# kije/gpu_raytracer

Hardware: AMD Instinct MI355X
Metric: Mrays/s (higher is better)
Workload: dtype f32

## Files before the change

gpu_raytracer_amd/csrc/rt_frame.cpp:

```cpp
#include "rt_internal.h"

#ifndef RT_SINGLE_PASS_MAX_NODES
#define RT_SINGLE_PASS_MAX_NODES 64u
#endif
#ifndef RT_WF_LANES_DEFAULT
#define RT_WF_LANES_DEFAULT 2
#endif

namespace rti {
DevCamera make_camera(const rt_camera& cam, float res_x, float res_y, bool wavefront) {
    DevCamera c;
    float wf, hf;
    if (wavefront) {
        wf = res_x;
        hf = res_y;
    } else {
        auto as_u32 = [](float f) -> uint32_t { return !(f > 0.0f) ? 0u : (f >= 4294967296.0f ? 0xFFFFFFFFu : (uint32_t)f); };
        wf = (float)as_u32(res_x);
        hf = (float)as_u32(res_y);
    }
    c.width_f = wf;
    c.height_f = hf;
    c.aspect = wf / hf;
    c.fov_scale = tanf(cam.fov * 0.5f * 3.14159265358979323846f / 180.0f);
// ... 311 lines not shown
    if (two) {
        HIPCHK(ctx, hipEventRecord(d.ev_start, d.stream));
        HIPCHK(ctx, hipStreamWaitEvent(d.stream2, d.ev_start, 0));
        HIPCHK(ctx, hipMemsetAsync(d.pipe.wf2.totals, 0, rt::WF_N_TOTALS * sizeof(unsigned long long), d.stream2));
    }
    d.pipe.wf.grids = d.pipe.wf2.grids = (f.flags & RT_FLAG_NO_SHADOW_GRID) ? nullptr : d.grids.table.get();
    const char* pe = std::getenv("RT_WF_PROBE");
    d.pipe.wf.probe = d.pipe.wf2.probe = pe ? (uint32_t)std::atoi(pe) : 0u;
    d.used_two_lanes = two;
    r = WfRun{};
    r.phase = WfRun::GENERATE;
    r.pipeline = true;
    r.dev = j;
    r.f = f;
    r.dsc = scene_for(ctx, d);
    r.batch = batch;
    r.n_blocks = n_blocks;
    r.two = two;
    r.beams = beams;
    return RT_OK;
}

struct WfLane { rt::WfBuffers w; hipStream_t st; };
WfLane lane_of(const DeviceState& d, const WfRun& r) {
    const bool second = r.two && (r.j & 1u);
    WfLane l{second ? d.pipe.wf2 : d.pipe.wf, second ? d.stream2 : d.stream};
    if (!r.beams) l.w.beam_count = nullptr;
    l.w.n_blocks = r.n_blocks;
    l.w.batch = r.batch;
    return l;
}
uint32_t batch_samples(const WfRun& r) { return std::min(r.batch, r.f.spp - r.first); }

int wf_step_generate(rt_ctx* ctx, DeviceState& d, WfRun& r, const WfLane& l) {
    HIPCHK(ctx, rt::wf_generate(r.dsc, r.f, l.w, targets_for(d, r.f), r.first, batch_samples(r), l.st));
    r.it = 0;
    r.phase = WfRun::BOUNCE;
    return RT_OK;
}

int wf_step_bounce(rt_ctx* ctx, DeviceState& d, WfRun& r, const WfLane& l, bool counters, std::vector<WfRun*>& polls) {
    hipEvent_t* gev = nullptr;
    if ((r.f.flags & RT_FLAG_STAGE_TIMES) && r.dev == 0 && rt::wf_runs_shadow_grid(r.f, l.w)) {
        if (d.stage_events.size() < (size_t)d.stage_events_used + 2) {
            hipEvent_t a = nullptr, b = nullptr;
            HIPCHK(ctx, hipEventCreate(&a));
            HIPCHK(ctx, hipEventCreate(&b));
            d.stage_events.push_back(a);
            d.stage_events.push_back(b);
        }
        gev = d.stage_events.data() + d.stage_events_used;
        d.stage_events_used += 2;
    }
    HIPCHK(ctx, rt::wf_bounce(r.dsc, r.f, l.w, r.it, batch_samples(r), counters, l.st, gev));
    if (r.it >= r.f.max_bounce) r.phase = WfRun::RESOLVE;
    else if ((r.it & 7u) == 7u) {
        HIPCHK(ctx, hipMemcpyAsync(&r.alive, l.w.counters + rt::WF_EXT_COUNT, 4, hipMemcpyDeviceToHost, l.st));
        r.poll_stream = l.st;
        polls.push_back(&r);
    } else r.it++;
    return RT_OK;
}

int wf_step_resolve(rt_ctx* ctx, DeviceState& d, WfRun& r, const WfLane& l) {
    const uint32_t n = batch_samples(r);
    if (r.two && r.j > 0) HIPCHK(ctx, hipStreamWaitEvent(l.st, d.ev_res[(r.j - 1u) & 1u], 0));
    HIPCHK(ctx, rt::wf_resolve(r.f, l.w, targets_for(d, r.f), n, r.first, r.first == 0, r.first + n >= r.f.spp, l.st));
    if (r.two) HIPCHK(ctx, hipEventRecord(d.ev_res[r.j & 1u], l.st));
    r.first += r.batch;
    r.j++;
    if (r.first < r.f.spp) {
        r.phase = WfRun::GENERATE;
        return RT_OK;
    }
    if (r.two) {
        HIPCHK(ctx, hipEventRecord(d.ev_join, d.stream2));
        HIPCHK(ctx, hipStreamWaitEvent(d.stream, d.ev_join, 0));
    }
    if (r.f.adaptive) HIPCHK(ctx, rt::launch_ad_image(r.f, targets_for(d, r.f), d.stream));
    HIPCHK(ctx, hipEventRecord(d.ev1, d.stream));
    r.phase = WfRun::DONE;
    return RT_OK;
}

struct FrameTotals {
    double kernel_ms = 0.0;
    uint64_t pixels = 0;
    unsigned long long segments = 0, camera = 0, continuation = 0, shadow = 0, node_visits = 0, tri_tests = 0;
    unsigned long long diag[RT_CNT_N_DIAG] = {0};
    unsigned long long grid_answered = 0, grid_entries = 0;
};

void add_counters(FrameTotals& t, const unsigned long long (&c)[RT_CNT_SLOTS]) {
    t.segments += c[RT_CNT_SEGMENTS], t.camera += c[RT_CNT_CAMERA], t.continuation += c[RT_CNT_CONTINUATION], t.shadow += c[RT_CNT_SHADOW];
    t.node_visits += c[RT_CNT_NODE_VISITS], t.tri_tests += c[RT_CNT_TRI_TESTS];
    for (int k = 0; k < RT_CNT_N_DIAG; k++) t.diag[k] += c[RT_CNT_DIAG + k];
}

void merge_lanes(unsigned long long (&t)[rt::WF_N_TOTALS], const unsigned long long (&t2)[rt::WF_N_TOTALS]) {
    for (int k = 0; k < rt::WF_N_TOTALS; k++) t[k] = k == rt::WF_TOTAL_STACK_MAX ? std::max(t[k], t2[k]) : t[k] + t2[k];
}

int add_totals(rt_ctx* ctx, FrameTotals& t, const unsigned long long (&w)[rt::WF_N_TOTALS]) {
    t.segments += w[rt::WF_TOTAL_CAMERA] + w[rt::WF_TOTAL_CONTINUATION] + w[rt::WF_TOTAL_SHADOW];
    t.camera += w[rt::WF_TOTAL_CAMERA], t.continuation += w[rt::WF_TOTAL_CONTINUATION], t.shadow += w[rt::WF_TOTAL_SHADOW];
    t.node_visits += w[rt::WF_TOTAL_NODE_VISITS], t.tri_tests += w[rt::WF_TOTAL_TRI_TESTS];
    if (w[rt::WF_TOTAL_ERROR] != 0)
// ... 273 lines not shown
```

gpu_raytracer_amd/csrc/wavefront.h:

```cpp
#ifndef RT_WAVEFRONT_H
#define RT_WAVEFRONT_H

#include <hip/hip_runtime.h>

#include "../../include/rt_hip.h"
#include "device_layout.h"
#include "shadow_grid.h"

namespace rt {

enum WfCounter : uint32_t {
    WF_EXT_COUNT = 0,
    WF_EXT_NEXT = 1,
    WF_SHADOW2_COUNT = 2,
    WF_SHADOW_COUNT = 3,
    WF_EXT_CURSOR = 4,
    WF_SHADOW_CURSOR = 5,
    WF_EXT_WINDOW = 6,
    WF_SHADOW_WINDOW = 7,
    WF_EXT_WINDOW_NEXT = 8,
    WF_SHADOW2_CURSOR = 9,
    WF_SHADOW2_WINDOW = 10,
    WF_UNUSED_11 = 11,
    WF_FB_COUNT = 12,
// ... 24 lines not shown
struct WfBuffers {
    float4* ray_o;
    float4* ray_d;
    float4* thr;
    float4* rad;
    float4* next_o;
    float4* next_d;
    float4* next_thr;
    float4* next_rad;
    float4* vtx;
    float4* sample_rad;
    uint32_t* pxy;
    uint32_t* q_ext[2];
    uint32_t* q_shadow;
    uint32_t* q_shadow2;
    const DevShadowGrid* grids;
    uint32_t* counters;
    unsigned long long* totals;
    float4* accum;
    uint32_t q_ext_cap;
    uint32_t q_shadow_cap;
    uint32_t state_cap;
    uint32_t* stack_ovf;
    uint32_t ovf_entries;
    uint32_t n_blocks;
    uint32_t batch;
    uint32_t capacity;
    uint32_t* beam_count;
    uint32_t* beam_ref;
    float* beam_dist;
    uint32_t probe;
};

#ifndef RT_BEAM_CAP
#define RT_BEAM_CAP 128u
#endif
#define RT_BEAM_OVERFLOW 0x80000000u
#ifndef RT_WF8_LDS_STACK
#define RT_WF8_LDS_STACK 8
#endif
#define RT_WF_MAX_LIGHTS 32u
#define RT_WF_ID_MASK 0x07FFFFFFu

uint32_t wf_shading_blocks();
size_t wf_state_slots(size_t paths);
size_t wf_state_slots_for(size_t paths, size_t producing_waves);
size_t wf_queue_slots(size_t max_entries, uint32_t per_lane);
size_t wf_queue_slots_for(size_t max_entries, uint32_t per_lane, size_t producing_waves);
uint32_t wf_pick_window(uint32_t iterations, uint32_t per_lane);
uint32_t wf_persistent_waves();
hipError_t wf_beams(const DevScene& sc, const DevFrame& fr, const WfBuffers& wb, hipStream_t s);
hipError_t wf_generate(const DevScene& sc, const DevFrame& fr, const WfBuffers& wb, const DevTargets& tg, uint32_t first_sample, uint32_t n_samples, hipStream_t s);
inline bool wf_runs_shadow_grid(const DevFrame& fr, const WfBuffers& wb) { return !(fr.flags & RT_FLAG_NO_SHADOWS) && wb.grids; }
hipError_t wf_bounce(const DevScene& sc, const DevFrame& fr, const WfBuffers& wb, uint32_t iteration, uint32_t n_samples, bool counters, hipStream_t s,
                     hipEvent_t* grid_events = nullptr);
hipError_t wf_resolve(const DevFrame& fr, const WfBuffers& wb, const DevTargets& tg, uint32_t n_samples, uint32_t first_sample, bool first_batch, bool last_batch,
                      hipStream_t s);

}
#endif
```

gpu_raytracer_amd/csrc/wavefront.hip:

```cpp
#include "wavefront.h"
#include <cstdlib>

#include <algorithm>

#include "device_common.h"
#include "shadow_grid_walk.h"

using namespace rtdev;

#ifndef RT_WF_REFILL
#define RT_WF_REFILL 16
#endif
#ifndef RT_WF_CHUNK
#define RT_WF_CHUNK 256
#endif
#ifndef RT_WF_ADAPTIVE_CHUNK
#define RT_WF_ADAPTIVE_CHUNK 1
#endif
#ifndef RT_WF_WINDOW
#define RT_WF_WINDOW 512
#endif
#ifndef RT_WF_BLOCK_MAJOR
#define RT_WF_BLOCK_MAJOR 1
#endif
// ... 20 lines not shown

#ifndef RT_WF_WINDOW_MAX
#define RT_WF_WINDOW_MAX 16384u
#endif
__host__ __device__ inline uint32_t wf_min_window(uint32_t per_lane) {
    uint32_t w = RT_WF_WINDOW;
    while (w < 128u * per_lane) w <<= 1;
    return w;
}
__host__ __device__ inline uint32_t pick_window(uint32_t iters, uint32_t per_lane) {
    const uint32_t most = iters * WAVE * per_lane;
    uint32_t w = wf_min_window(per_lane);
    while (w < most / 4u && w < RT_WF_WINDOW_MAX) w <<= 1;
    return w;
}
struct OutWindow {
    uint32_t next, end;
};
#define WF_SENTINEL 0xFFFFFFFFu
__device__ __forceinline__ void window_close(uint32_t* __restrict__ queue, OutWindow& w) {
    for (uint32_t i = w.next + (threadIdx.x & 63u); i < w.end; i += WAVE) queue[i] = WF_SENTINEL;
    w.next = w.end;
}
#define WF_NO_SLOT 0xFFFFFFFFu
__device__ __forceinline__ uint32_t window_reserve(uint32_t* __restrict__ queue, uint32_t* __restrict__ counter, OutWindow& w, uint32_t window,
                                                  uint32_t mine, uint32_t incl, uint32_t total, uint32_t capacity, unsigned long long* __restrict__ error) {
    if (w.next + total > w.end) {
        window_close(queue, w);
        uint32_t base = 0;
        if ((threadIdx.x & 63u) == 0) base = atomicAdd(counter, window);
        base = __shfl(base, 0, WAVE);
        if (base > capacity || window > capacity - base) {
            if ((threadIdx.x & 63u) == 0) atomicOr(error, 1ull);
            w.next = w.end = 0u;
            return WF_NO_SLOT;
        }
        w.next = base;
        w.end = base + window;
    }
    const uint32_t at = w.next + incl - mine;
    w.next += total;
    return at;
}
__device__ __forceinline__ uint32_t wave_incl_scan(uint32_t v) {
    const uint32_t lane = threadIdx.x & 63u;
#pragma unroll
    for (int off = 1; off < WAVE; off <<= 1) {
        const uint32_t u = __shfl_up(v, off, WAVE);
        if ((int)lane >= off) v += u;
    }
    return v;
}

template <bool AD>
__global__ __launch_bounds__(256) void k_wf_generate(DevFrame fr, rt::WfBuffers wb, DevTargets tg, uint32_t first_sample, uint32_t n_slots_blocks) {
    const uint32_t lane = threadIdx.x & 63u;
    const uint32_t n_waves = gridDim.x * 4u, wave = blockIdx.x * 4u + (threadIdx.x >> 6);
    OutWindow win = {0u, 0u};
    uint32_t real = 0;
    const uint32_t window = pick_window((n_slots_blocks + n_waves - 1u) / n_waves, 1u);
    if (blockIdx.x == 0 && threadIdx.x == 0) {
        wb.counters[rt::WF_EXT_WINDOW] = window;
        if (wb.beam_count) wb.counters[rt::WF_FB_COUNT] = wb.beam_count[wb.n_blocks] * (n_slots_blocks / max(1u, wb.n_blocks)) * WAVE;
    }
    const uint32_t n_samples = n_slots_blocks / max(1u, wb.n_blocks);
    for (uint32_t sb = wave; sb < n_slots_blocks; sb += n_waves) {
#if RT_WF_BLOCK_MAJOR
        const uint32_t b = sb / n_samples, k = sb - b * n_samples;
#else
        const uint32_t k = sb / wb.n_blocks, b = sb - k * wb.n_blocks;
#endif
        PixelCoord px = block_pixel_at(fr, AD ? fr.ad_blocks[b] : b, lane);
        uint32_t base = fr.sample_base;
        if (AD) {
            px.valid = px.valid && ad_lane_active(fr, fr.ad_blocks[b], lane);
            if (px.valid) base = ad_load(fr, tg, (size_t)px.y * fr.width + px.x).n;
        }
        const uint32_t p = sb * WAVE + lane;
        if (px.valid) {
            V3 o, d;
            const SimpleRng rng = ext_sample_ray(fr.cam, fr.width, fr.frame_seed, fr.jitter, px.x, px.y, base + first_sample + k, true, o, d);
            wb.ray_o[p] = make_float4(o.x, o.y, o.z, 0.0f);
            wb.ray_d[p] = make_float4(d.x, d.y, d.z, __uint_as_float(p));
            wb.thr[p] = make_float4(1.0f, 1.0f, 1.0f, __uint_as_float(3u));
            wb.rad[p] = make_float4(0.0f, 0.0f, 0.0f, __uint_as_float(rng.seed));
            wb.pxy[p] = px.x | (px.y << 16);
        } else {
            wb.pxy[p] = 0xFFFFFFFFu;
            wb.sample_rad[p] = make_float4(0.0f, 0.0f, 0.0f, 0.0f);
        }
        const uint32_t mine = px.valid ? 1u : 0u;
        const uint32_t incl = wave_incl_scan(mine), total = __shfl(incl, WAVE - 1, WAVE);
        if (total) {
            const uint32_t at = window_reserve(wb.q_ext[0], &wb.counters[rt::WF_EXT_COUNT], win, window, mine, incl, total, wb.q_ext_cap, &wb.totals[rt::WF_TOTAL_ERROR]);
            if (mine && at != WF_NO_SLOT) wb.q_ext[0][at] = p;
            real += mine;
        }
        if (wb.beam_count) {
            const uint32_t bc = wb.beam_count[b];
            if (bc & RT_BEAM_OVERFLOW) wb.q_ext[1][((size_t)(bc & ~RT_BEAM_OVERFLOW) * n_samples + k) * WAVE + lane] = px.valid ? p : WF_SENTINEL;
        }
    }
    window_close(wb.q_ext[0], win);
    const unsigned long long r = wave_sum(real);
    if (lane == 0 && r) atomicAdd(&wb.totals[rt::WF_TOTAL_CAMERA], r);
}

#ifndef RT_WF8_LDS_STACK
#define RT_WF8_LDS_STACK 8
#endif
#ifndef RT_WF8_MIN_WAVES
#define RT_WF8_MIN_WAVES 6
#endif
#ifndef RT_WF8_LEAF_THRESHOLD
#define RT_WF8_LEAF_THRESHOLD 24
#endif
#define WF8_KIND_T 0x80000000u
#define WF8_NONE 0xFFFFFFFFu

#define WF_NO_VERTEX 0xFFFFFFFFu
#define WF_END_SKY 0u
#define WF_END_MAGENTA 1u
__device__ __forceinline__ uint32_t wf_all_lights(uint32_t n_lights) { return n_lights >= RT_WF_MAX_LIGHTS ? 0xFFFFFFFFu : (1u << n_lights) - 1u; }
__device__ __forceinline__ void wf_store_vertex(const DevScene& sc, const rt::WfBuffers& wb, uint32_t id, bool found, V3 point, V3 normal, uint32_t material_id) {
    float4* __restrict__ rec = wb.vtx + 2 * (size_t)id;
    if (found && material_id < sc.n_materials) {
        rec[0] = make_float4(point.x, point.y, point.z, __uint_as_float(material_id));
        rec[1] = make_float4(normal.x, normal.y, normal.z, __uint_as_float(wf_all_lights(sc.n_lights)));
    } else {
        rec[0] = make_float4(__uint_as_float(found ? WF_END_MAGENTA : WF_END_SKY), 0.0f, 0.0f, __uint_as_float(WF_NO_VERTEX));
    }
}

template <bool COUNT, bool ANY>
__global__ __launch_bounds__(WAVE, RT_WF8_MIN_WAVES) void k_wf_trace(DevScene sc, rt::WfBuffers wb, const uint32_t* __restrict__ queue, uint32_t count_slot,
                                                    uint32_t cursor_slot, uint32_t window_slot) {
    extern __shared__ uint32_t s_mem8[];
    if (wb.totals[rt::WF_TOTAL_ERROR] != 0ull) return;
    const uint32_t lane = threadIdx.x;
    uint2* __restrict__ stack = reinterpret_cast<uint2*>(s_mem8) + lane;
    uint8_t* __restrict__ lut = reinterpret_cast<uint8_t*>(s_mem8 + RT_WF8_LDS_STACK * 2 * WAVE);
    for (uint32_t e = lane; e < 2048u; e += WAVE) {
        const uint32_t oct = e >> 8, m = e & 255u;
        uint32_t best = 0u, best_key = 99u;
        for (uint32_t i = 0; i < 8u; i++)
            if (((m >> i) & 1u) && (i ^ oct) < best_key) best_key = i ^ oct, best = i;
        lut[e] = (uint8_t)best;
    }
    __syncthreads();
    uint2* __restrict__ ovf = reinterpret_cast<uint2*>(wb.stack_ovf) + (size_t)blockIdx.x * wb.ovf_entries * WAVE + lane;
    const uint4* __restrict__ nodes = reinterpret_cast<const uint4*>(sc.nodes);
    const uint32_t count = wb.counters[count_slot];
// ... 349 lines not shown
    for (uint32_t l0 = 0; l0 < n_leaf && !overflow; l0 += WAVE) {
        const uint32_t li = l0 + lane;
        uint32_t first = 0, count = 0;
        if (li < n_leaf) {
            first = s_leaf[li];
            count = sc.tris[first].leaf_count;
        }
        for (uint32_t k = 0; k < RT_DEV_LEAF_STRIDE; k++) {
            bool keep = false;
            float dist = 0.0f;
            if (k < count) {
                const DevTri& t = sc.tris[first + k];
                float lo[3], hi[3];
                for (int a = 0; a < 3; a++) {
                    const float va = t.v0[a], vb = t.v0[a] + t.e1[a], vc = t.v0[a] + t.e2[a];
                    lo[a] = fminf(va, fminf(vb, vc));
                    hi[a] = fmaxf(va, fmaxf(vb, vc));
                    const float pad = (fabsf(lo[a]) + fabsf(hi[a])) * 2.0e-6f + 1.0e-30f;
                    lo[a] -= pad;
                    hi[a] += pad;
                }
                keep = !RT_BEAM_TRI_CULL || !(lo[0] <= hi[0] && lo[1] <= hi[1] && lo[2] <= hi[2]) || !beam_outside(bp, lo, hi);
                dist = beam_box_distance(bp.o, lo, hi);
                if (!(dist >= 0.0f)) dist = 0.0f;
            }
            const unsigned long long mk = __ballot(keep);
            const uint32_t pos = n_tri + (uint32_t)__popcll(mk & lower);
            if (keep && pos < RT_BEAM_CAP) {
                s_ref[pos] = first + k;
                s_dist[pos] = dist;
            }
            n_tri += (uint32_t)__popcll(mk);
        }
        overflow = n_tri > RT_BEAM_CAP;
    }
    __syncthreads();
    if (overflow) {
        if (lane == 0) wb.beam_count[b] = RT_BEAM_OVERFLOW | atomicAdd(&wb.beam_count[wb.n_blocks], 1u);
        return;
    }
    for (uint32_t i = lane; i < n_tri; i += WAVE) {
        const float di = s_dist[i];
        uint32_t rank = 0;
        for (uint32_t j = 0; j < n_tri; j++) {
            const float dj = s_dist[j];
            rank += (dj < di || (dj == di && j < i)) ? 1u : 0u;
        }
        wb.beam_ref[(size_t)b * RT_BEAM_CAP + rank] = s_ref[i];
        wb.beam_dist[(size_t)b * RT_BEAM_CAP + rank] = di;
    }
    if (lane == 0) wb.beam_count[b] = n_tri;
}

template <bool COUNT>
__global__ __launch_bounds__(WAVE) void k_wf_trace_camera(DevScene sc, rt::WfBuffers wb, uint32_t n_samples) {
    extern __shared__ uint4 s_cam[];
    if (wb.totals[rt::WF_TOTAL_ERROR] != 0ull) return;
    const uint32_t lane = threadIdx.x;
    float* s_d = reinterpret_cast<float*>(s_cam + RT_BEAM_CAP * 3u);
    Counts cnt = {0u, 0u};
    const uint32_t chunks = (n_samples + RT_BEAM_SAMPLES_PER_WAVE - 1u) / RT_BEAM_SAMPLES_PER_WAVE;
    for (uint32_t item = blockIdx.x; item < wb.n_blocks * chunks; item += gridDim.x) {
        const uint32_t b = item / chunks, k_first = (item - b * chunks) * RT_BEAM_SAMPLES_PER_WAVE, k_end = min(n_samples, k_first + RT_BEAM_SAMPLES_PER_WAVE);
        const uint32_t n_list = (uint32_t)__builtin_amdgcn_readfirstlane((int)wb.beam_count[b]);
        if (n_list & RT_BEAM_OVERFLOW) continue;
        {
            __syncthreads();
            for (uint32_t i = lane; i < n_list; i += WAVE) {
                const uint32_t slot = wb.beam_ref[(size_t)b * RT_BEAM_CAP + i];
                const uint4* __restrict__ rec = reinterpret_cast<const uint4*>(sc.tris + slot);
                const uint4 q0 = rec[0], q1 = rec[1], q2 = rec[2];
                s_cam[3u * i] = q0;
                s_cam[3u * i + 1u] = q1;
                s_cam[3u * i + 2u] = make_uint4(q2.x, q2.y, q2.z, slot);
                s_d[i] = wb.beam_dist[(size_t)b * RT_BEAM_CAP + i];
            }
            __syncthreads();
        }
        for (uint32_t k = k_first; k < k_end; k++) {
            const uint32_t sb = RT_WF_BLOCK_MAJOR ? b * n_samples + k : k * wb.n_blocks + b;
            const uint32_t p = sb * WAVE + lane;
            const bool valid = wb.pxy[p] != 0xFFFFFFFFu;
            if (__ballot(valid) == 0ull) continue;
            V3 o = v3(0.0f, 0.0f, 0.0f), d = v3(0.0f, 0.0f, 1.0f);
            if (valid) {
                float4 ro = wb.ray_o[p], rd = wb.ray_d[p];
                RT_KEEP4_EARLY(ro);
                RT_KEEP4_EARLY(rd);
                o = f4v(ro);
                d = f4v(rd);
            }
            Hit hit;
            hit.t = valid ? RT_F32_MAX : -1.0f;
            hit.prim = RT_PRIM_MISS;
            hit.slot = 0;
            uint32_t hit_i = 0;
            if (valid) test_spheres(sc, o, d, hit, RT_MIN_RAY_DISTANCE);
            {
                for (uint32_t i = 0; i < n_list; i++) {
                    if (RT_BEAM_EARLY_OUT && __ballot(s_d[i] < hit.t) == 0ull) break;
                    const uint4 q0 = s_cam[3u * i], q1 = s_cam[3u * i + 1u], q2 = s_cam[3u * i + 2u];
                    if (COUNT && valid) cnt.tris++;
                    float t = 0.0f;
                    const bool inside = moller_trumbore(v3(__uint_as_float(q0.x), __uint_as_float(q0.y), __uint_as_float(q0.z)), v3(__uint_as_float(q0.w), __uint_as_float(q1.x), __uint_as_float(q1.y)),
                                                        v3(__uint_as_float(q1.z), __uint_as_float(q1.w), __uint_as_float(q2.x)), o, d, t);
                    const uint32_t prim = q2.z;
                    const bool accept = inside && t > RT_MIN_RAY_DISTANCE && (t < hit.t || (t == hit.t && prim < hit.prim && hit.prim < RT_PRIM_SPHERE_FLAG));
                    hit.t = accept ? t : hit.t;
                    hit.prim = accept ? prim : hit.prim;
                    hit.slot = accept ? q2.w : hit.slot;
                    hit_i = accept ? i : hit_i;
                }
            }
            if (COUNT && wb.probe == 2u && valid) {
                Hit h2;
                h2.t = RT_F32_MAX;
                h2.prim = RT_PRIM_MISS;
                h2.slot = 0;
                Counts c2 = {0u, 0u};
                test_spheres(sc, o, d, h2, RT_MIN_RAY_DISTANCE);
                traverse<false, false>(sc, o, d, reinterpret_cast<uint2*>(s_cam + RT_BEAM_CAP * 4u) + lane, h2, c2, RT_MIN_RAY_DISTANCE);
                if (h2.prim != hit.prim || h2.t != hit.t) {
                    if (atomicAdd(&wb.totals[rt::WF_TOTAL_EMPTY_VISITS], 1ull) == 0ull) {
                        wb.totals[rt::WF_TOTAL_NODE_STEPS] = b;
                        wb.totals[rt::WF_TOTAL_LEAF_STEPS] = ((unsigned long long)hit.prim << 32) | h2.prim;
                        wb.totals[rt::WF_TOTAL_LEAF_LANES] = ((unsigned long long)__float_as_uint(hit.t) << 32) | __float_as_uint(h2.t);
                        wb.totals[rt::WF_TOTAL_LEAF_TRIPS] = ((unsigned long long)n_list << 32) | h2.slot;
                        wb.totals[rt::WF_TOTAL_REFILLS] = p;
                    }
                }
            }
            if (valid) {
                const bool found = hit.prim != RT_PRIM_MISS;
                V3 hp = v3(0.0f, 0.0f, 0.0f), normal = hp;
                uint32_t material_id = 0;
                if (found) {
                    hp = o + d * hit.t;
                    if (hit.prim & RT_PRIM_SPHERE_FLAG) {
                        surface_at(sc, true, hit.prim & ~RT_PRIM_SPHERE_FLAG, hp, normal, material_id);
                    } else {
                        const uint4 q0 = s_cam[3u * hit_i], q1 = s_cam[3u * hit_i + 1u], q2 = s_cam[3u * hit_i + 2u];
                        const V3 e1 = v3(__uint_as_float(q0.w), __uint_as_float(q1.x), __uint_as_float(q1.y));
                        const V3 e2 = v3(__uint_as_float(q1.z), __uint_as_float(q1.w), __uint_as_float(q2.x));
// ... 219 lines not shown
                }
            }
            if (to_grids) {
                n_shadow += (uint32_t)__popc(mask);
                continue;
            }
#if RT_WF_SHADOW_LIGHT_MAJOR
            uint32_t total = 0;
            for (uint32_t li = 0; li < sc.n_lights; li++) total += (uint32_t)__popcll(__ballot((mask >> li) & 1u));
            if (total) {
                uint32_t at = window_reserve(wb.q_shadow, &wb.counters[rt::WF_SHADOW_COUNT], win, window, 0u, 0u, total, wb.q_shadow_cap, &wb.totals[rt::WF_TOTAL_ERROR]);
                n_shadow += (uint32_t)__popc(mask);
                const unsigned long long below = (1ull << (threadIdx.x & 63u)) - 1ull;
                for (uint32_t li = 0; at != WF_NO_SLOT && li < sc.n_lights; li++) {
                    const bool want = (mask >> li) & 1u;
                    const unsigned long long b = __ballot(want);
                    if (want) wb.q_shadow[at + (uint32_t)__popcll(b & below)] = id | (li << 27);
                    at += (uint32_t)__popcll(b);
                }
            }
#else
            const uint32_t mine = (uint32_t)__popc(mask);
            const uint32_t incl = wave_incl_scan(mine), total = __shfl(incl, WAVE - 1, WAVE);
            if (total) {
                uint32_t at = window_reserve(wb.q_shadow, &wb.counters[rt::WF_SHADOW_COUNT], win, window, mine, incl, total, wb.q_shadow_cap, &wb.totals[rt::WF_TOTAL_ERROR]);
                n_shadow += mine;
                while (mask && at != WF_NO_SLOT) {
                    const uint32_t li = (uint32_t)__ffs((int)mask) - 1u;
                    mask &= mask - 1u;
                    wb.q_shadow[at++] = id | (li << 27);
                }
            }
#endif
        }
    }
    window_close(wb.q_shadow, win);
    const unsigned long long ns = wave_sum(n_shadow);
    if ((threadIdx.x & 63u) == 0 && ns) atomicAdd(&wb.totals[rt::WF_TOTAL_SHADOW], ns);
}

__global__ void k_wf_advance(rt::WfBuffers wb) {
    if (threadIdx.x != 0 || blockIdx.x != 0) return;
    uint32_t* c = wb.counters;
    c[rt::WF_EXT_COUNT] = c[rt::WF_EXT_NEXT];
    c[rt::WF_EXT_WINDOW] = c[rt::WF_EXT_WINDOW_NEXT];
    c[rt::WF_EXT_NEXT] = 0;
    c[rt::WF_SHADOW_COUNT] = 0;
    c[rt::WF_SHADOW2_COUNT] = 0;
    c[rt::WF_SHADOW2_CURSOR] = 0;
    c[rt::WF_EXT_CURSOR] = 0;
    c[rt::WF_SHADOW_CURSOR] = 0;
}

__global__ __launch_bounds__(256, RT_WF_SHADE_WAVES) void k_wf_finish(DevScene sc, DevFrame fr, rt::WfBuffers wb, const uint32_t* __restrict__ queue,
                                                  uint32_t* __restrict__ next_queue) {
    __shared__ DevLight s_lights[RT_WF_MAX_LIGHTS];
    if (wb.totals[rt::WF_TOTAL_ERROR] != 0ull) return;
    stage_lights(s_lights, sc);
    const uint32_t count = wb.counters[rt::WF_EXT_COUNT];
    const bool shadows = (fr.flags & RT_FLAG_NO_SHADOWS) == 0;
    const uint32_t stride = gridDim.x * blockDim.x;
    OutWindow win = {0u, 0u};
    uint32_t n_cont = 0;
    const uint32_t window = pick_window((count + stride - 1u) / stride, 1u);
    if (blockIdx.x == 0 && threadIdx.x == 0) wb.counters[rt::WF_EXT_WINDOW_NEXT] = window;
    uint32_t id_next = blockIdx.x * blockDim.x + threadIdx.x < count ? queue[blockIdx.x * blockDim.x + threadIdx.x] : WF_SENTINEL;
    for (uint32_t base = blockIdx.x * blockDim.x; base < count; base += stride) {
        bool cont = false;
        V3 norigin = v3(0.0f, 0.0f, 0.0f), ndir = norigin, throughput = norigin, radiance = norigin;
        uint32_t next_tw = 0, rng_seed = 0, ndir_origin = 0;
        const uint32_t id = id_next;
        const uint32_t i_next = base + stride + threadIdx.x;
        id_next = i_next < count ? queue[i_next] : WF_SENTINEL;
        float4 vp = make_float4(0.0f, 0.0f, 0.0f, __uint_as_float(0xFFFFFFFFu));
        float4 vn = vp, th = vp, ra = vp, rdin = vp;
        if (id != WF_SENTINEL) {
            vp = wb.vtx[2 * (size_t)id];
            vn = wb.vtx[2 * (size_t)id + 1];
            th = wb.thr[id];
            ra = wb.rad[id];
            rdin = wb.ray_d[id];
            RT_KEEP4(vp);
            RT_KEEP4(vn);
            RT_KEEP4(th);
            RT_KEEP4(ra);
            RT_KEEP4(rdin);
        }
        const uint32_t vis = __float_as_uint(vn.w);
        if (id != WF_SENTINEL && __float_as_uint(vp.w) == WF_NO_VERTEX) {
            const V3 end = __float_as_uint(vp.x) == WF_END_SKY ? RT_SKY() : RT_MAGENTA();
            wf_end_path(wb, __float_as_uint(rdin.w), f4v(ra) + end * f4v(th));
        } else if (__float_as_uint(vp.w) != WF_NO_VERTEX) {
            const V3 point = f4v(vp), normal = f4v(vn);
            const uint32_t material_id = __float_as_uint(vp.w);
            const uint32_t origin = __float_as_uint(rdin.w);
            const DevMaterial m = load_material(sc, material_id);
            throughput = f4v(th), radiance = f4v(ra);
            const uint32_t tw = __float_as_uint(th.w);
            uint32_t channel = tw & 0xFFu;
            const uint32_t depth = tw >> 8;
            SimpleRng rng = {__float_as_uint(ra.w)};
            const bool terminal = depth >= fr.max_bounce;
            const V3 lighting = ext_light_sum(s_lights, sc.n_lights, m, point, normal, terminal, shadows, [&](uint32_t li, V3, float) { return ((vis >> li) & 1u) != 0u; });
            const float tf = ext_leave_vertex(m, lighting, terminal, throughput, radiance);
            if (terminal || !ext_scatter(m, point, normal, f4v(rdin), tf, depth, rng, channel, throughput, norigin, ndir)) {
                wf_end_path(wb, origin, radiance);
            } else {
                cont = true;
                next_tw = channel | ((depth + 1u) << 8);
                rng_seed = rng.seed;
                ndir_origin = origin;
            }
        }
        const uint32_t mine = cont ? 1u : 0u;
        const uint32_t incl = wave_incl_scan(mine), total = __shfl(incl, WAVE - 1, WAVE);
        if (total) {
            const uint32_t at = window_reserve(next_queue, &wb.counters[rt::WF_EXT_NEXT], win, window, mine, incl, total, wb.state_cap, &wb.totals[rt::WF_TOTAL_ERROR]);
            if (cont && at != WF_NO_SLOT) {
                wb.next_o[at] = make_float4(norigin.x, norigin.y, norigin.z, 0.0f);
                wb.next_d[at] = make_float4(ndir.x, ndir.y, ndir.z, __uint_as_float(ndir_origin));
                wb.next_thr[at] = make_float4(throughput.x, throughput.y, throughput.z, __uint_as_float(next_tw));
                wb.next_rad[at] = make_float4(radiance.x, radiance.y, radiance.z, __uint_as_float(rng_seed));
                next_queue[at] = at;
            }
            n_cont += mine;
        }
    }
    window_close(next_queue, win);
    const unsigned long long nc = wave_sum(n_cont);
    if ((threadIdx.x & 63u) == 0 && nc) atomicAdd(&wb.totals[rt::WF_TOTAL_CONTINUATION], nc);
}

template <bool AD>
__global__ __launch_bounds__(WAVE) void k_wf_resolve(DevFrame fr, rt::WfBuffers wb, DevTargets tg, uint32_t n_samples, uint32_t first_sample, uint32_t first_batch,
                                                     uint32_t last_batch) {
    const uint32_t lane = threadIdx.x, b = blockIdx.x;
    const uint32_t q = b * WAVE + lane;
    if (AD) {
        const uint32_t ob = fr.ad_blocks[b];
// ... 63 lines not shown
}
size_t wf_state_slots_for(size_t paths, size_t waves) {
    static_assert(RT_WF_WINDOW > 64, "a closed window holds at least RT_WF_WINDOW - 63 real entries");
    const size_t closed = (paths * RT_WF_WINDOW + (RT_WF_WINDOW - 64)) / (RT_WF_WINDOW - 63);
    const size_t stride = std::max<size_t>(1, waves) * WAVE;
    auto after = [&](size_t consumed) {
        const size_t iters = std::min<size_t>((consumed + stride - 1) / stride, 0xFFFFFFFFull / (WAVE * 4u));
        const size_t producing = std::min(std::min(waves, (consumed + WAVE - 1) / WAVE), paths);
        return closed + producing * (size_t)pick_window((uint32_t)iters, 1u);
    };
    size_t c = after(paths), most = paths;
    for (int depth = 0; depth < 64; depth++) {
        const size_t n = after(c);
        most = std::max(most, n);
        if (n == c) break;
        c = n;
    }
    return most;
}
size_t wf_state_slots(size_t paths) { return wf_state_slots_for(paths, (size_t)wf_shading_blocks() * 4); }
size_t wf_queue_slots(size_t max_entries, uint32_t per_lane) { return wf_queue_slots_for(max_entries, per_lane, (size_t)wf_shading_blocks() * 4); }
uint32_t wf_pick_window(uint32_t iters, uint32_t per_lane) { return pick_window(iters, per_lane); }
uint32_t wf_persistent_waves() { return (uint32_t)(cu_count() * RT_WF_WAVES_PER_CU); }
static uint32_t trace_waves_per_cu(uint32_t path_slots) {
    static const int forced = [] { const char* e = std::getenv("RT_WF_WAVES_PER_CU"); const int v = e ? std::atoi(e) : 0; return v > 0 && v <= RT_WF_WAVES_PER_CU ? v : 0; }();
    if (forced) return (uint32_t)forced;
    return path_slots >= (24u << 20) ? (uint32_t)RT_WF_WAVES_PER_CU : RT_WF_WAVES_SMALL;
}

hipError_t wf_beams(const DevScene& sc, const DevFrame& fr, const WfBuffers& wb, hipStream_t s) {
    if (!wb.beam_count || wb.n_blocks == 0) return hipSuccess;
    const hipError_t e = hipMemsetAsync(wb.beam_count + wb.n_blocks, 0, sizeof(uint32_t), s);
    if (e != hipSuccess) return e;
    if (fr.adaptive) hipLaunchKernelGGL(k_wf_beams<true>, dim3(wb.n_blocks), dim3(WAVE), 0, s, sc, fr, wb);
    else hipLaunchKernelGGL(k_wf_beams<false>, dim3(wb.n_blocks), dim3(WAVE), 0, s, sc, fr, wb);
    return hipGetLastError();
}

hipError_t wf_generate(const DevScene&, const DevFrame& fr, const WfBuffers& wb, const DevTargets& tg, uint32_t first_sample, uint32_t n_samples, hipStream_t s) {
    hipError_t e = hipMemsetAsync(wb.counters, 0, WF_N_COUNTERS * sizeof(uint32_t), s);
    if (e != hipSuccess) return e;
    if (wb.n_blocks == 0 || n_samples == 0) return hipSuccess;
    if (fr.adaptive) hipLaunchKernelGGL(k_wf_generate<true>, dim3(wf_shading_blocks()), dim3(256), 0, s, fr, wb, tg, first_sample, n_samples * wb.n_blocks);
    else hipLaunchKernelGGL(k_wf_generate<false>, dim3(wf_shading_blocks()), dim3(256), 0, s, fr, wb, tg, first_sample, n_samples * wb.n_blocks);
    return hipGetLastError();
}

template <bool COUNT, bool ANY>
static void launch_trace(const DevScene& sc, const WfBuffers& wb, const uint32_t* q, uint32_t count_slot, uint32_t cursor_slot, uint32_t window_slot, hipStream_t s) {
    const size_t lds = (size_t)RT_WF8_LDS_STACK * WAVE * sizeof(uint2) + 2048;
    hipLaunchKernelGGL((k_wf_trace<COUNT, ANY>), dim3((uint32_t)cu_count() * trace_waves_per_cu(wb.capacity)), dim3(WAVE), lds, s, sc, wb, q, count_slot, cursor_slot, window_slot);
}

hipError_t wf_bounce(const DevScene& sc, const DevFrame& fr, const WfBuffers& wb_in, uint32_t iteration, uint32_t n_samples, bool counters, hipStream_t s, hipEvent_t* grid_events) {
    const dim3 sgrid(wf_shading_blocks()), sblock(256);
    WfBuffers wb = wb_in;
    if (iteration & 1u) {
        std::swap(wb.ray_o, wb.next_o);
        std::swap(wb.ray_d, wb.next_d);
        std::swap(wb.thr, wb.next_thr);
        std::swap(wb.rad, wb.next_rad);
    }
    uint32_t* cur_q = wb.q_ext[iteration & 1u];
    uint32_t* next_q = wb.q_ext[(iteration + 1u) & 1u];
    if (iteration == 0 && wb.beam_count && n_samples && wb.n_blocks) {
        const dim3 lgrid(std::min<uint32_t>(wb.n_blocks * ((n_samples + RT_BEAM_SAMPLES_PER_WAVE - 1u) / RT_BEAM_SAMPLES_PER_WAVE), (uint32_t)cu_count() * 96u));
        const size_t list_lds = (size_t)RT_BEAM_CAP * (3 * sizeof(uint4) + sizeof(float)), walk_lds = (size_t)std::max(1u, sc.stack_entries) * WAVE * sizeof(uint2);
        if (counters) {
            hipLaunchKernelGGL((k_wf_trace_camera<true>), lgrid, dim3(WAVE), wb.probe == 2u ? (size_t)RT_BEAM_CAP * 64 + walk_lds : list_lds, s, sc, wb, n_samples);
            launch_trace<true, false>(sc, wb, wb.q_ext[1], WF_FB_COUNT, WF_FB_CURSOR, WF_SHADOW2_WINDOW, s);
        } else {
            hipLaunchKernelGGL((k_wf_trace_camera<false>), lgrid, dim3(WAVE), list_lds, s, sc, wb, n_samples);
            launch_trace<false, false>(sc, wb, wb.q_ext[1], WF_FB_COUNT, WF_FB_CURSOR, WF_SHADOW2_WINDOW, s);
        }
    } else if (counters) launch_trace<true, false>(sc, wb, cur_q, WF_EXT_COUNT, WF_EXT_CURSOR, WF_EXT_WINDOW, s);
    else launch_trace<false, false>(sc, wb, cur_q, WF_EXT_COUNT, WF_EXT_CURSOR, WF_EXT_WINDOW, s);
    if ((fr.flags & RT_FLAG_NO_SHADOWS) == 0 && !(RT_WF_GRID_MASK && wf_runs_shadow_grid(fr, wb))) hipLaunchKernelGGL(k_wf_shade, sgrid, sblock, 0, s, sc, wb, (const uint32_t*)cur_q);
    if (wf_runs_shadow_grid(fr, wb)) {
        const dim3 ggrid((uint32_t)(cu_count() * RT_WF_GRID_BLOCKS_PER_CU));
        if (grid_events) (void)hipEventRecord(grid_events[0], s);
        if (counters) hipLaunchKernelGGL(k_wf_shadow_grid<true>, ggrid, dim3(256), 0, s, sc, wb, (const uint32_t*)cur_q);
        else hipLaunchKernelGGL(k_wf_shadow_grid<false>, ggrid, dim3(256), 0, s, sc, wb, (const uint32_t*)cur_q);
        if (grid_events) (void)hipEventRecord(grid_events[1], s);
        if (counters) launch_trace<true, true>(sc, wb, wb.q_shadow2, WF_SHADOW2_COUNT, WF_SHADOW2_CURSOR, WF_SHADOW2_WINDOW, s);
        else launch_trace<false, true>(sc, wb, wb.q_shadow2, WF_SHADOW2_COUNT, WF_SHADOW2_CURSOR, WF_SHADOW2_WINDOW, s);
    } else if ((fr.flags & RT_FLAG_NO_SHADOWS) == 0) {
        if (counters) launch_trace<true, true>(sc, wb, wb.q_shadow, WF_SHADOW_COUNT, WF_SHADOW_CURSOR, WF_SHADOW_WINDOW, s);
        else launch_trace<false, true>(sc, wb, wb.q_shadow, WF_SHADOW_COUNT, WF_SHADOW_CURSOR, WF_SHADOW_WINDOW, s);
    }
    hipLaunchKernelGGL(k_wf_finish, sgrid, sblock, 0, s, sc, fr, wb, (const uint32_t*)cur_q, next_q);
    hipLaunchKernelGGL(k_wf_advance, dim3(1), dim3(1), 0, s, wb);
    return hipGetLastError();
}

hipError_t wf_resolve(const DevFrame& fr, const WfBuffers& wb, const DevTargets& tg, uint32_t n_samples, uint32_t first_sample, bool first_batch, bool last_batch,
                      hipStream_t s) {
    if (wb.n_blocks == 0) return hipSuccess;
    if (fr.adaptive)
        hipLaunchKernelGGL(k_wf_resolve<true>, dim3(wb.n_blocks), dim3(WAVE), 0, s, fr, wb, tg, n_samples, first_sample, first_batch ? 1u : 0u, last_batch ? 1u : 0u);
    else
        hipLaunchKernelGGL(k_wf_resolve<false>, dim3(wb.n_blocks), dim3(WAVE), 0, s, fr, wb, tg, n_samples, first_sample, first_batch ? 1u : 0u, last_batch ? 1u : 0u);
    return hipGetLastError();
}

}
```

Baseline: 3436.

## Recompute depth-0 camera ray state instead of storing it in generate

For non-adaptive frames, the generate kernel no longer writes ray origin, direction, throughput and radiance for each camera path. It writes them only for beam-overflow blocks that still go through the generic trace. The camera-trace kernel and the depth-0 finish kernel instead rebuild the ray and RNG seed from the pixel coordinate and sample index. This trades global-memory stores and reloads for extra ALU work. It risks inconsistency if any other iteration-0 consumer, such as the shade or shadow-grid kernels, still reads the unwritten thr/rad/ray_d buffers.

```diff
diff --git a/gpu_raytracer_amd/csrc/rt_frame.cpp b/gpu_raytracer_amd/csrc/rt_frame.cpp
--- a/gpu_raytracer_amd/csrc/rt_frame.cpp
+++ b/gpu_raytracer_amd/csrc/rt_frame.cpp
@@ -387,7 +387,7 @@
         gev = d.stage_events.data() + d.stage_events_used;
         d.stage_events_used += 2;
     }
-    HIPCHK(ctx, rt::wf_bounce(r.dsc, r.f, l.w, r.it, batch_samples(r), counters, l.st, gev));
+    HIPCHK(ctx, rt::wf_bounce(r.dsc, r.f, l.w, r.it, batch_samples(r), r.first, counters, l.st, gev));
     if (r.it >= r.f.max_bounce) r.phase = WfRun::RESOLVE;
     else if ((r.it & 7u) == 7u) {
         HIPCHK(ctx, hipMemcpyAsync(&r.alive, l.w.counters + rt::WF_EXT_COUNT, 4, hipMemcpyDeviceToHost, l.st));
diff --git a/gpu_raytracer_amd/csrc/wavefront.h b/gpu_raytracer_amd/csrc/wavefront.h
--- a/gpu_raytracer_amd/csrc/wavefront.h
+++ b/gpu_raytracer_amd/csrc/wavefront.h
@@ -100,8 +100,8 @@
 hipError_t wf_beams(const DevScene& sc, const DevFrame& fr, const WfBuffers& wb, hipStream_t s);
 hipError_t wf_generate(const DevScene& sc, const DevFrame& fr, const WfBuffers& wb, const DevTargets& tg, uint32_t first_sample, uint32_t n_samples, hipStream_t s);
 inline bool wf_runs_shadow_grid(const DevFrame& fr, const WfBuffers& wb) { return !(fr.flags & RT_FLAG_NO_SHADOWS) && wb.grids; }
-hipError_t wf_bounce(const DevScene& sc, const DevFrame& fr, const WfBuffers& wb, uint32_t iteration, uint32_t n_samples, bool counters, hipStream_t s,
-                     hipEvent_t* grid_events = nullptr);
+hipError_t wf_bounce(const DevScene& sc, const DevFrame& fr, const WfBuffers& wb, uint32_t iteration, uint32_t n_samples, uint32_t first_sample, bool counters,
+                     hipStream_t s, hipEvent_t* grid_events = nullptr);
 hipError_t wf_resolve(const DevFrame& fr, const WfBuffers& wb, const DevTargets& tg, uint32_t n_samples, uint32_t first_sample, bool first_batch, bool last_batch,
                       hipStream_t s);
 
diff --git a/gpu_raytracer_amd/csrc/wavefront.hip b/gpu_raytracer_amd/csrc/wavefront.hip
--- a/gpu_raytracer_amd/csrc/wavefront.hip
+++ b/gpu_raytracer_amd/csrc/wavefront.hip
@@ -96,6 +96,27 @@
     return v;
 }
 
+__device__ __forceinline__ uint32_t wf_slot_block(uint32_t b, uint32_t k, uint32_t n_samples, uint32_t n_blocks) {
+    return RT_WF_BLOCK_MAJOR ? b * n_samples + k : k * n_blocks + b;
+}
+__device__ __forceinline__ void wf_slot_split(uint32_t sb, uint32_t n_samples, uint32_t n_blocks, uint32_t& b, uint32_t& k) {
+#if RT_WF_BLOCK_MAJOR
+    b = sb / n_samples, k = sb - b * n_samples;
+#else
+    k = sb / n_blocks, b = sb - k * n_blocks;
+#endif
+}
+#define WF_DEPTH0_TW 3u
+__device__ __forceinline__ SimpleRng wf_camera_state(const DevFrame& fr, uint32_t first_sample, uint32_t k, uint32_t pxy, V3& o, V3& d) {
+    return ext_sample_ray(fr.cam, fr.width, fr.frame_seed, fr.jitter, pxy & 0xFFFFu, pxy >> 16, fr.sample_base + first_sample + k, true, o, d);
+}
+__device__ __forceinline__ SimpleRng wf_camera_state_of(const DevFrame& fr, uint32_t n_samples, uint32_t n_blocks, uint32_t first_sample, uint32_t p, uint32_t pxy,
+                                                        V3& o, V3& d) {
+    uint32_t b, k;
+    wf_slot_split(p / WAVE, n_samples, n_blocks, b, k);
+    return wf_camera_state(fr, first_sample, k, pxy, o, d);
+}
+
 template <bool AD>
 __global__ __launch_bounds__(256) void k_wf_generate(DevFrame fr, rt::WfBuffers wb, DevTargets tg, uint32_t first_sample, uint32_t n_slots_blocks) {
     const uint32_t lane = threadIdx.x & 63u;
@@ -109,26 +130,32 @@
     }
     const uint32_t n_samples = n_slots_blocks / max(1u, wb.n_blocks);
     for (uint32_t sb = wave; sb < n_slots_blocks; sb += n_waves) {
-#if RT_WF_BLOCK_MAJOR
-        const uint32_t b = sb / n_samples, k = sb - b * n_samples;
-#else
-        const uint32_t k = sb / wb.n_blocks, b = sb - k * wb.n_blocks;
-#endif
+        uint32_t b, k;
+        wf_slot_split(sb, n_samples, wb.n_blocks, b, k);
         PixelCoord px = block_pixel_at(fr, AD ? fr.ad_blocks[b] : b, lane);
         uint32_t base = fr.sample_base;
         if (AD) {
             px.valid = px.valid && ad_lane_active(fr, fr.ad_blocks[b], lane);
             if (px.valid) base = ad_load(fr, tg, (size_t)px.y * fr.width + px.x).n;
         }
+        const uint32_t bc = wb.beam_count ? wb.beam_count[b] : RT_BEAM_OVERFLOW;
         const uint32_t p = sb * WAVE + lane;
         if (px.valid) {
-            V3 o, d;
-            const SimpleRng rng = ext_sample_ray(fr.cam, fr.width, fr.frame_seed, fr.jitter, px.x, px.y, base + first_sample + k, true, o, d);
-            wb.ray_o[p] = make_float4(o.x, o.y, o.z, 0.0f);
-            wb.ray_d[p] = make_float4(d.x, d.y, d.z, __uint_as_float(p));
-            wb.thr[p] = make_float4(1.0f, 1.0f, 1.0f, __uint_as_float(3u));
-            wb.rad[p] = make_float4(0.0f, 0.0f, 0.0f, __uint_as_float(rng.seed));
-            wb.pxy[p] = px.x | (px.y << 16);
+            const uint32_t pxy = px.x | (px.y << 16);
+            if (AD) {
+                V3 o, d;
+                const SimpleRng rng = ext_sample_ray(fr.cam, fr.width, fr.frame_seed, fr.jitter, px.x, px.y, base + first_sample + k, true, o, d);
+                wb.ray_o[p] = make_float4(o.x, o.y, o.z, 0.0f);
+                wb.ray_d[p] = make_float4(d.x, d.y, d.z, __uint_as_float(p));
+                wb.thr[p] = make_float4(1.0f, 1.0f, 1.0f, __uint_as_float(WF_DEPTH0_TW));
+                wb.rad[p] = make_float4(0.0f, 0.0f, 0.0f, __uint_as_float(rng.seed));
+            } else if (bc & RT_BEAM_OVERFLOW) {
+                V3 o, d;
+                wf_camera_state(fr, first_sample, k, pxy, o, d);
+                wb.ray_o[p] = make_float4(o.x, o.y, o.z, 0.0f);
+                wb.ray_d[p] = make_float4(d.x, d.y, d.z, __uint_as_float(p));
+            }
+            wb.pxy[p] = pxy;
         } else {
             wb.pxy[p] = 0xFFFFFFFFu;
             wb.sample_rad[p] = make_float4(0.0f, 0.0f, 0.0f, 0.0f);
@@ -141,7 +168,6 @@
             real += mine;
         }
         if (wb.beam_count) {
-            const uint32_t bc = wb.beam_count[b];
             if (bc & RT_BEAM_OVERFLOW) wb.q_ext[1][((size_t)(bc & ~RT_BEAM_OVERFLOW) * n_samples + k) * WAVE + lane] = px.valid ? p : WF_SENTINEL;
         }
     }
@@ -597,8 +623,8 @@
     if (lane == 0) wb.beam_count[b] = n_tri;
 }
 
-template <bool COUNT>
-__global__ __launch_bounds__(WAVE) void k_wf_trace_camera(DevScene sc, rt::WfBuffers wb, uint32_t n_samples) {
+template <bool COUNT, bool IMPLICIT>
+__global__ __launch_bounds__(WAVE) void k_wf_trace_camera(DevScene sc, DevFrame fr, rt::WfBuffers wb, uint32_t n_samples, uint32_t first_sample) {
     extern __shared__ uint4 s_cam[];
     if (wb.totals[rt::WF_TOTAL_ERROR] != 0ull) return;
     const uint32_t lane = threadIdx.x;
@@ -623,17 +649,21 @@
             __syncthreads();
         }
         for (uint32_t k = k_first; k < k_end; k++) {
-            const uint32_t sb = RT_WF_BLOCK_MAJOR ? b * n_samples + k : k * wb.n_blocks + b;
-            const uint32_t p = sb * WAVE + lane;
-            const bool valid = wb.pxy[p] != 0xFFFFFFFFu;
+            const uint32_t p = wf_slot_block(b, k, n_samples, wb.n_blocks) * WAVE + lane;
+            const uint32_t pxy = wb.pxy[p];
+            const bool valid = pxy != 0xFFFFFFFFu;
             if (__ballot(valid) == 0ull) continue;
             V3 o = v3(0.0f, 0.0f, 0.0f), d = v3(0.0f, 0.0f, 1.0f);
             if (valid) {
-                float4 ro = wb.ray_o[p], rd = wb.ray_d[p];
-                RT_KEEP4_EARLY(ro);
-                RT_KEEP4_EARLY(rd);
-                o = f4v(ro);
-                d = f4v(rd);
+                if (IMPLICIT) {
+                    wf_camera_state(fr, first_sample, k, pxy, o, d);
+                } else {
+                    float4 ro = wb.ray_o[p], rd = wb.ray_d[p];
+                    RT_KEEP4_EARLY(ro);
+                    RT_KEEP4_EARLY(rd);
+                    o = f4v(ro);
+                    d = f4v(rd);
+                }
             }
             Hit hit;
             hit.t = valid ? RT_F32_MAX : -1.0f;
@@ -959,8 +989,9 @@
     c[rt::WF_SHADOW_CURSOR] = 0;
 }
 
+template <bool IMPLICIT>
 __global__ __launch_bounds__(256, RT_WF_SHADE_WAVES) void k_wf_finish(DevScene sc, DevFrame fr, rt::WfBuffers wb, const uint32_t* __restrict__ queue,
-                                                  uint32_t* __restrict__ next_queue) {
+                                                  uint32_t* __restrict__ next_queue, uint32_t n_samples, uint32_t first_sample) {
     __shared__ DevLight s_lights[RT_WF_MAX_LIGHTS];
     if (wb.totals[rt::WF_TOTAL_ERROR] != 0ull) return;
     stage_lights(s_lights, sc);
@@ -984,14 +1015,25 @@
         if (id != WF_SENTINEL) {
             vp = wb.vtx[2 * (size_t)id];
             vn = wb.vtx[2 * (size_t)id + 1];
-            th = wb.thr[id];
-            ra = wb.rad[id];
-            rdin = wb.ray_d[id];
-            RT_KEEP4(vp);
-            RT_KEEP4(vn);
-            RT_KEEP4(th);
-            RT_KEEP4(ra);
-            RT_KEEP4(rdin);
+            if (IMPLICIT) {
+                const uint32_t pxy = wb.pxy[id];
+                RT_KEEP4(vp);
+                RT_KEEP4(vn);
+                V3 o, d;
+                const SimpleRng rng0 = wf_camera_state_of(fr, n_samples, wb.n_blocks, first_sample, id, pxy, o, d);
+                th = make_float4(1.0f, 1.0f, 1.0f, __uint_as_float(WF_DEPTH0_TW));
+                ra = make_float4(0.0f, 0.0f, 0.0f, __uint_as_float(rng0.seed));
+                rdin = make_float4(d.x, d.y, d.z, __uint_as_float(id));
+            } else {
+                th = wb.thr[id];
+                ra = wb.rad[id];
+                rdin = wb.ray_d[id];
+                RT_KEEP4(vp);
+                RT_KEEP4(vn);
+                RT_KEEP4(th);
+                RT_KEEP4(ra);
+                RT_KEEP4(rdin);
+            }
         }
         const uint32_t vis = __float_as_uint(vn.w);
         if (id != WF_SENTINEL && __float_as_uint(vp.w) == WF_NO_VERTEX) {
@@ -1161,8 +1203,10 @@
     hipLaunchKernelGGL((k_wf_trace<COUNT, ANY>), dim3((uint32_t)cu_count() * trace_waves_per_cu(wb.capacity)), dim3(WAVE), lds, s, sc, wb, q, count_slot, cursor_slot, window_slot);
 }
 
-hipError_t wf_bounce(const DevScene& sc, const DevFrame& fr, const WfBuffers& wb_in, uint32_t iteration, uint32_t n_samples, bool counters, hipStream_t s, hipEvent_t* grid_events) {
+hipError_t wf_bounce(const DevScene& sc, const DevFrame& fr, const WfBuffers& wb_in, uint32_t iteration, uint32_t n_samples, uint32_t first_sample, bool counters,
+                     hipStream_t s, hipEvent_t* grid_events) {
     const dim3 sgrid(wf_shading_blocks()), sblock(256);
+    const bool implicit = !fr.adaptive;
     WfBuffers wb = wb_in;
     if (iteration & 1u) {
         std::swap(wb.ray_o, wb.next_o);
@@ -1176,10 +1220,13 @@
         const dim3 lgrid(std::min<uint32_t>(wb.n_blocks * ((n_samples + RT_BEAM_SAMPLES_PER_WAVE - 1u) / RT_BEAM_SAMPLES_PER_WAVE), (uint32_t)cu_count() * 96u));
         const size_t list_lds = (size_t)RT_BEAM_CAP * (3 * sizeof(uint4) + sizeof(float)), walk_lds = (size_t)std::max(1u, sc.stack_entries) * WAVE * sizeof(uint2);
         if (counters) {
-            hipLaunchKernelGGL((k_wf_trace_camera<true>), lgrid, dim3(WAVE), wb.probe == 2u ? (size_t)RT_BEAM_CAP * 64 + walk_lds : list_lds, s, sc, wb, n_samples);
+            const size_t lds = wb.probe == 2u ? (size_t)RT_BEAM_CAP * 64 + walk_lds : list_lds;
+            if (implicit) hipLaunchKernelGGL((k_wf_trace_camera<true, true>), lgrid, dim3(WAVE), lds, s, sc, fr, wb, n_samples, first_sample);
+            else hipLaunchKernelGGL((k_wf_trace_camera<true, false>), lgrid, dim3(WAVE), lds, s, sc, fr, wb, n_samples, first_sample);
             launch_trace<true, false>(sc, wb, wb.q_ext[1], WF_FB_COUNT, WF_FB_CURSOR, WF_SHADOW2_WINDOW, s);
         } else {
-            hipLaunchKernelGGL((k_wf_trace_camera<false>), lgrid, dim3(WAVE), list_lds, s, sc, wb, n_samples);
+            if (implicit) hipLaunchKernelGGL((k_wf_trace_camera<false, true>), lgrid, dim3(WAVE), list_lds, s, sc, fr, wb, n_samples, first_sample);
+            else hipLaunchKernelGGL((k_wf_trace_camera<false, false>), lgrid, dim3(WAVE), list_lds, s, sc, fr, wb, n_samples, first_sample);
             launch_trace<false, false>(sc, wb, wb.q_ext[1], WF_FB_COUNT, WF_FB_CURSOR, WF_SHADOW2_WINDOW, s);
         }
     } else if (counters) launch_trace<true, false>(sc, wb, cur_q, WF_EXT_COUNT, WF_EXT_CURSOR, WF_EXT_WINDOW, s);
@@ -1197,7 +1244,8 @@
         if (counters) launch_trace<true, true>(sc, wb, wb.q_shadow, WF_SHADOW_COUNT, WF_SHADOW_CURSOR, WF_SHADOW_WINDOW, s);
         else launch_trace<false, true>(sc, wb, wb.q_shadow, WF_SHADOW_COUNT, WF_SHADOW_CURSOR, WF_SHADOW_WINDOW, s);
     }
-    hipLaunchKernelGGL(k_wf_finish, sgrid, sblock, 0, s, sc, fr, wb, (const uint32_t*)cur_q, next_q);
+    if (iteration == 0 && implicit) hipLaunchKernelGGL(k_wf_finish<true>, sgrid, sblock, 0, s, sc, fr, wb, (const uint32_t*)cur_q, next_q, n_samples, first_sample);
+    else hipLaunchKernelGGL(k_wf_finish<false>, sgrid, sblock, 0, s, sc, fr, wb, (const uint32_t*)cur_q, next_q, n_samples, first_sample);
     hipLaunchKernelGGL(k_wf_advance, dim3(1), dim3(1), 0, s, wb);
     return hipGetLastError();
 }
```

Result: faster. 3496 (median of 6 runs) (+1.7%).
